# psteinb/libmultiviewnative

Hardware: AMD Instinct MI355X
Metric: RL iterations/sec on 512^3 f32, 6 views (higher is better)
Workload: dtype f32

## Files before the change

### libmultiviewnative_amd/csrc/mvn_backend_emu.cpp

```cpp
#ifndef MVN_HOST_EMU
#error "mvn_backend_emu.cpp is only for the MVN_HOST_EMU test build"
#endif

#include <atomic>
#include <chrono>
#include <cstdlib>
#include <cstring>
#include <map>
#include <memory>
#include <mutex>
#include <stdexcept>
#include <string>
#include <vector>

#include "mvn_backend.hpp"
#include "mvn_fixed_geom.hpp"
#include "mvn_wave_rows.hpp"

namespace mvn {
namespace be {

#define MVN_DISPATCH_T(T_, CALL)                                   \
  switch (T_) {                                                    \
    case 16: { constexpr int TT = 16; CALL; } break;               \
// ... 181 lines not shown
          case MVN_EPI_DIVIDE: fx_rows_run<H, 1, MVN_EPI_DIVIDE, Ctx, true>(p, t, ntiles, l, *ctx); break;
          case MVN_EPI_UPDATE: fx_rows_run<H, 1, MVN_EPI_UPDATE, Ctx, true>(p, t, ntiles, l, *ctx); break;
          case MVN_EPI_UPDATE_STATS: fx_rows_run_stats<H, 1, SCtx, true>(p, t, ntiles, l, *sctx); break;
          case MVN_EPI_DELTA: fx_rows_run<H, 1, MVN_EPI_DELTA, Ctx, true>(p, t, ntiles, l, *ctx); break;
          default: fx_rows_run<H, 1, MVN_EPI_STORE, Ctx, true>(p, t, ntiles, l, *ctx); break;
        }
      } else {
        switch (p.epi.mode) {
          case MVN_EPI_DIVIDE: fx_rows_run<H, 2, MVN_EPI_DIVIDE, Ctx, true>(p, t, ntiles, l, *ctx); break;
          case MVN_EPI_UPDATE: fx_rows_run<H, 2, MVN_EPI_UPDATE, Ctx, true>(p, t, ntiles, l, *ctx); break;
          case MVN_EPI_UPDATE_STATS: fx_rows_run_stats<H, 2, SCtx, true>(p, t, ntiles, l, *sctx); break;
          default: fx_rows_run<H, 2, MVN_EPI_STORE, Ctx, true>(p, t, ntiles, l, *ctx); break;
        }
      }
    }
  }
}

static std::atomic<long> g_mid_fused_launches{0};
long mid_fused_launch_count() { return g_mid_fused_launches.load(); }

template <int K>
static void emu_mid_fused(const MidFusedParams& p) {
  typedef FxCtx<MfRegs<K>, MF_NT> Ctx;
  const long blocks = mf_blocks(p);
#pragma omp parallel
  {
    std::vector<cfloat> lds(MF_LDS_CFLOATS + 8);
    std::unique_ptr<Ctx> ctx(new Ctx());
#pragma omp for schedule(static)
    for (long b = 0; b < blocks; ++b) mf_body<K>(p, b, lds.data(), *ctx);
  }
}
#define MVN_MF_TAP_COUNTS(X) X(1) X(3) X(5) X(7) X(9) X(11) X(13) X(15) X(17) X(19) X(21) X(23) X(25) X(27) X(29) X(31)
void launch_mid_fused(const MidFusedParams& p, stream_t) {
  mf_check(p);
  if (p.mode == MF_TAPS) {
    typedef FxCtx<MfRegs<1>, MF_NT> Ctx;
    const long blocks = mf_blocks(p);
#pragma omp parallel
    {
      std::vector<cfloat> lds(MF_LDS_CFLOATS + 8);
      std::unique_ptr<Ctx> ctx(new Ctx());
#pragma omp for schedule(static)
      for (long b = 0; b < blocks; ++b) mf_taps_body(p, b, lds.data(), *ctx);
    }
    return;
// ... 362 lines not shown
```

### libmultiviewnative_amd/csrc/mvn_kernels.hip

```cpp
#include <hip/hip_runtime.h>

#include <atomic>
#include <cstdio>
#include <cstdlib>
#include <cstring>
#include <map>
#include <mutex>
#include <tuple>
#include <stdexcept>
#include <string>

#include "mvn_backend.hpp"
#include "mvn_fixed_geom.hpp"
#include "mvn_wave_rows.hpp"

#define HIP_CHECK(expr)                                                                      \
  do {                                                                                       \
    hipError_t _e = (expr);                                                                  \
    if (_e != hipSuccess)                                                                    \
      throw std::runtime_error(std::string("HIP error '") + hipGetErrorString(_e) + "' at " + \
                               __FILE__ + ":" + std::to_string(__LINE__) + " (" #expr ")");  \
  } while (0)

template <bool EVEN, int T>
// ... 63 lines not shown
  Ctx ctx;
  ctx.tid = (int)threadIdx.x;
  if constexpr (EPI == MVN_EPI_UPDATE_STATS)
    fx_rows_run_stats<H, 1, Ctx, LINES>(p, (long)blockIdx.x, (long)gridDim.x, (cfloat*)mvn_smem, ctx);
  else
    fx_rows_run<H, 1, EPI, Ctx, LINES>(p, (long)blockIdx.x, (long)gridDim.x, (cfloat*)mvn_smem, ctx);
}

template <int H, int EPI, bool LINES = false>
__global__ void __launch_bounds__(FxRowsCfg<H>::NT) kx_rows_c2r_r2c(const RowsParams p0) {
  extern __shared__ __attribute__((aligned(16))) char mvn_smem[];
  RowsParams p = p0;
  mvn_arm_poison(p.epi);
  typedef FxCtx<FxRowsRegsFor<H, EPI>, FxRowsCfg<H>::NT> Ctx;
  Ctx ctx;
  ctx.tid = (int)threadIdx.x;
  if constexpr (EPI == MVN_EPI_UPDATE_STATS)
    fx_rows_run_stats<H, 2, Ctx, LINES>(p, (long)blockIdx.x, (long)gridDim.x, (cfloat*)mvn_smem, ctx);
  else
    fx_rows_run<H, 2, EPI, Ctx, LINES>(p, (long)blockIdx.x, (long)gridDim.x, (cfloat*)mvn_smem, ctx);
}

template <int K>
__global__ void __launch_bounds__(MF_NT) kf_mid(const MidFusedParams p) {
  extern __shared__ __attribute__((aligned(16))) char mvn_smem[];
  FxCtx<MfRegs<K>, MF_NT> ctx;
  ctx.tid = (int)threadIdx.x;
  mf_body<K>(p, (long)blockIdx.x, (cfloat*)mvn_smem, ctx);
}
__global__ void __launch_bounds__(MF_NT) kf_mid_taps(const MidFusedParams p) {
  extern __shared__ __attribute__((aligned(16))) char mvn_smem[];
  FxCtx<MfRegs<1>, MF_NT> ctx;
  ctx.tid = (int)threadIdx.x;
  mf_taps_body(p, (long)blockIdx.x, (cfloat*)mvn_smem, ctx);
}

template <int MODE, int EPI>
__global__ void __launch_bounds__(WrCfg::NT, 4) kw_rows(const RowsParams p0) {
  extern __shared__ __attribute__((aligned(16))) char mvn_smem[];
  RowsParams p = p0;
  if (MODE != MVN_WR_R2C) mvn_arm_poison(p.epi);
  FxCtx<WrRegs, WrCfg::NT> ctx;
  ctx.tid = (int)threadIdx.x;
  wr_rows_body<MODE, EPI>(p, (long)blockIdx.x, (long)gridDim.x, (cfloat*)mvn_smem, ctx);
}

template <int N, int MODE>
__global__ void __launch_bounds__((FxStridedSel<N, MODE>::NT), (FxStridedSel<N, MODE>::WAVES))
    kx_strided(const StridedParams p, const StridedParams rider, unsigned main_grid) {
// ... 653 lines not shown
  }
  if (nblocks > 0x7fffffffL) throw std::invalid_argument("mvn: grid size out of range");
  switch (mvn_dim0_taps_template(p.k)) {
#define X(K) case K: hipLaunchKernelGGL(kd_dim0<K>, dim3((unsigned)nblocks), dim3(MVN_D0_WG), lds, hs(s), p, (unsigned)main_blocks); break;
    MVN_D0_TAP_COUNTS(X)
#undef X
    default: throw std::invalid_argument("mvn: no direct dim0 kernel for this tap count");
  }
  HIP_CHECK(hipGetLastError());
}

#define MVN_MF_TAP_COUNTS(X) X(1) X(3) X(5) X(7) X(9) X(11) X(13) X(15) X(17) X(19) X(21) X(23) X(25) X(27) X(29) X(31)
void launch_mid_fused(const MidFusedParams& p, stream_t s) {
  mf_check(p);
  const long nblocks = mf_blocks(p);
  if (nblocks < 1 || nblocks > 0x7fffffffL) throw std::invalid_argument("mvn: grid size out of range");
  const size_t lds = sizeof(cfloat) * (size_t)MF_LDS_CFLOATS;
  if (p.mode == MF_TAPS) {
    launch_pass(kf_mid_taps, p, nblocks, MF_NT, lds, s);
    return;
  }
  ++g_mid_fused_launches;
  switch (mvn_dim0_taps_template(p.k)) {
#define X(K) case K: launch_pass(kf_mid<K>, p, nblocks, MF_NT, lds, s); break;
    MVN_MF_TAP_COUNTS(X)
#undef X
    default: throw std::invalid_argument("mvn: no fused middle pass for this tap count");
  }
}

static unsigned flat_grid(size_t n, int block) {
  size_t g = (n + (size_t)block - 1) / (size_t)block;
  const size_t cap = (size_t)device_cu_count() * 8;
  if (g > cap) g = cap;
  if (g < 1) g = 1;
  return (unsigned)g;
}

void launch_scatter_psf(const float* kernel, int k0, int k1, int k2, float* target, int D0,
                        int D1, int D2, long pitch, float scale, stream_t s) {
  const size_t total = (size_t)k0 * k1 * k2;
  hipLaunchKernelGGL(k_scatter_psf, dim3(flat_grid(total, 256)), dim3(256), 0, hs(s), kernel, k0,
                     k1, k2, target, D0, D1, D2, pitch, scale);
  HIP_CHECK(hipGetLastError());
}

void launch_copy3d(float* dst, long drow, long dplane, const float* src, long srow, long splane,
// ... 55 lines not shown
```

### libmultiviewnative_amd/csrc/mvn_mid_fused.hpp

```cpp
#pragma once

#include <stdexcept>

#include "mvn_dim0_direct.hpp"
#include "mvn_wave_rows.hpp"

#if defined(__HIPCC__) && !defined(MVN_HOST_EMU)
#define MF_WPHASE(ctx, ...)                                         \
  {                                                                 \
    const int tid = (ctx).tid;                                      \
    auto& r = (ctx).regs;                                           \
    (void)r;                                                        \
    __VA_ARGS__;                                                    \
  }                                                                 \
  __builtin_amdgcn_fence(__ATOMIC_SEQ_CST, "wavefront", "local");   \
  __builtin_amdgcn_wave_barrier();
#else
#define MF_WPHASE(ctx, ...) MVN_PHASE(ctx, __VA_ARGS__)
#endif

#define MF_N1 512
#define MF_NT 512
#define MF_LINES 8
#define MF_PITCH 576
#define MF_BUF (MF_LINES * MF_PITCH)
#define MF_TWL 512
#define MF_LDS_CFLOATS (4 * MF_BUF + MF_TWL)

struct MidFusedParams {
  const cfloat* in;
  cfloat* out;
  const cfloat* taps;
  int kd;
  const cfloat* tw;
  int d0, H;
  int k, h;
  int seg;
  int mode;
  int packed;
  int zbeg, zcount;
  unsigned* poison;
  unsigned poison_epoch;
  int n_peers;
  unsigned* const* poison_peers;
};
enum { MF_CONV = 0, MF_TAPS = 1 };
enum { MF_DC_NONE = 0, MF_DC_LOW = 1, MF_DC_HIGH = 2, MF_DC_SELF = 3 };

constexpr int mf_slots(int K) { return (K + 7) / 8 * 8; }

template <int K>
struct MfRegs {
  cfloat tap[K];
  cfloat w[mf_slots(K)];
  cfloat xr[8];
  cfloat t[8];
  cfloat bad;
  cfloat t2[8];
  cfloat xn[2], xp[2];
  int dcmode, qm, cpar;
};

inline long mf_pieces(const MidFusedParams& P) { return (P.seg > 0 && P.zcount <= 0) ? (P.d0 + P.seg - 1) / P.seg : 1; }
inline long mf_blocks(const MidFusedParams& P) { return P.mode == MF_TAPS ? (long)P.H * ((P.d0 + MF_LINES - 1) / MF_LINES) : (long)P.H * mf_pieces(P); }

MVN_HD void mf_job(const MidFusedParams& P, long block, int& c, int& z0, int& nout) {
  const long piece = block / P.H;
  c = (int)(block - piece * P.H);
  if (P.zcount > 0) {
    z0 = P.zbeg;
    nout = P.zcount;
  } else if (P.seg > 0) {
    z0 = (int)(piece * P.seg);
    nout = P.d0 - z0 < P.seg ? P.d0 - z0 : P.seg;
  } else {
    z0 = 0;
    nout = P.d0;
  }
}

MVN_HD int mf_tap_plane(const MidFusedParams& P, int j) {
  const int p = j - P.h;
  return p < 0 ? p + P.kd : p;
}

inline void mf_check(const MidFusedParams& P) {
  const bool taps_mode = P.mode == MF_TAPS;
  if (!P.in || !P.out || !P.tw || P.d0 < 1 || P.H < 1 || (long)P.d0 * P.H * MF_N1 >= (1L << 31) * 4 || P.seg < 0)
    throw std::invalid_argument("mvn: fused middle pass: bad arguments");
  if (P.zcount < 0 || P.zbeg < 0 || P.zbeg + P.zcount > P.d0 || P.n_peers < 0 || P.n_peers > MVN_D0_MAX_PEERS ||
      (P.n_peers > 0 && !P.poison_peers))
    throw std::invalid_argument("mvn: fused middle pass: bad plane range or peers");
  if (!taps_mode && (!P.taps || P.in == P.out || P.k < 1 || mvn_dim0_taps_template(P.k) > 31 || P.h != P.k / 2 || P.kd < P.k))
    throw std::invalid_argument("mvn: fused middle pass called outside its range");
}

MVN_HD int mf_in_plane(const MidFusedParams& P, int z0, int n) {
  int z = (z0 - P.h + n) % P.d0;
  return z < 0 ? z + P.d0 : z;
}

template <int K>
MVN_HD void mf_fetch(const MidFusedParams& P, MfRegs<K>& r, int c, int z0, int batch, int nsteps, int tid) {
  const int wv = tid >> 6, l = tid & 63;
  const int n = batch * MF_LINES + wv;
  if (n >= nsteps) return;
  const cfloat* src = P.in + ((long)mf_in_plane(P, z0, n) * P.H + c) * MF_N1 + l;
#pragma unroll
  for (int m = 0; m < 8; ++m) r.xr[m] = src[64 * m];
}

template <int K>
MVN_HD void mf_setup(const MidFusedParams& P, MfRegs<K>& r, int c, int z0, int nsteps, int tid) {
  r.bad = cmake(0.f, 0.f);
  r.dcmode = MF_DC_NONE;
  r.qm = r.cpar = 0;
#pragma unroll
  for (int j = 0; j < K; ++j) r.tap[j] = j < P.k ? P.taps[((long)mf_tap_plane(P, j) * P.H + c) * MF_N1 + tid] : cmake(0.f, 0.f);
#pragma unroll
  for (int s = 0; s < mf_slots(K); ++s) r.w[s] = cmake(0.f, 0.f);
  mf_fetch<K>(P, r, c, z0, 0, nsteps, tid);
}

MVN_HD cfloat mf_cmul(cfloat a, cfloat w) {
#if defined(MVN_PACKED)
  cfloat t, r;
  MVN_PK2(t, "v_pk_mul_f32", a, w, "op_sel_hi:[0,1]");
  MVN_PK3(r, "v_pk_fma_f32", a, w, t, "op_sel:[1,1,0] op_sel_hi:[1,0,1] neg_lo:[0,1,0]");
  return r;
#else
  return cmul(a, w);
#endif
}
MVN_HD cfloat mf_cmulc(cfloat a, cfloat w) {
#if defined(MVN_PACKED)
  cfloat t, r;
  MVN_PK2(t, "v_pk_mul_f32", a, w, "op_sel_hi:[0,1] neg_hi:[0,1]");
  MVN_PK3(r, "v_pk_fma_f32", a, w, t, "op_sel:[1,1,0] op_sel_hi:[1,0,1]");
  return r;
#else
  return cmulc(a, w);
#endif
}

MVN_HD void mf_build_twiddles(const MidFusedParams& P, cfloat* twl, int tid) {
  if (tid < 448) {
    const int m = tid / 64 + 1, l = tid & 63;
    twl[tid] = P.tw[l * m];
  } else if (tid < 448 + 56) {
    const int e = tid - 448, m = e / 8 + 1, j = e & 7;
    twl[tid] = P.tw[8 * j * m];
  }
}
MVN_HD cfloat mf_tw0(const cfloat* twl, int l, int m) { return twl[(m - 1) * 64 + l]; }
MVN_HD cfloat mf_tw1(const cfloat* twl, int l, int m) { return twl[448 + (m - 1) * 8 + (l & 7)]; }

template <int K>
MVN_HD void mf_fwd0(MfRegs<K>& r, cfloat* buf, int tid) {
  const int wv = tid >> 6, l = tid & 63;
  cfloat* line = buf + wv * MF_PITCH;
  cfloat a[8];
#pragma unroll
  for (int m = 0; m < 8; ++m) a[m] = r.xr[m];
  dftR<8, -1>(a);
#pragma unroll
  for (int m = 1; m < 8; ++m) a[m] = mf_cmul(a[m], r.t2[m]);
#pragma unroll
  for (int m = 0; m < 8; ++m) line[72 * m + l] = a[m];
}
template <int K>
MVN_HD void mf_tw0_ahead(MfRegs<K>& r, const cfloat* twl, int tid) {
  const int l = tid & 63;
#pragma unroll
  for (int m = 1; m < 8; ++m) r.t2[m] = mf_tw0(twl, l, m);
}
template <int K>
MVN_HD void mf_fwd1_r(MfRegs<K>& r, const cfloat* buf, int tid) {
  const int wv = tid >> 6, l = tid & 63;
  const cfloat* p = buf + wv * MF_PITCH + 72 * (l >> 3) + (l & 7);
#pragma unroll
  for (int m = 0; m < 8; ++m) r.t[m] = p[8 * m];
}
template <int K>
MVN_HD void mf_fwd1_c(MfRegs<K>& r, const cfloat* twl, int tid) {
  const int l = tid & 63;
  (void)l;
  dftR<8, -1>(r.t);
#pragma unroll
  for (int m = 1; m < 8; ++m) r.t[m] = mf_cmul(r.t[m], mf_tw1(twl, l, m));
}
template <int K>
MVN_HD void mf_fwd1_r2(MfRegs<K>& r, const cfloat* buf, int tid) {
  const int wv = tid >> 6, l = tid & 63;
  const cfloat* p = buf + wv * MF_PITCH + 72 * (l >> 3) + (l & 7);
#pragma unroll
  for (int m = 0; m < 8; ++m) r.t2[m] = p[8 * m];
}
template <int K>
MVN_HD void mf_fwd1_c2(MfRegs<K>& r, const cfloat* twl, int tid) {
  const int l = tid & 63;
  (void)l;
  dftR<8, -1>(r.t2);
#pragma unroll
  for (int m = 1; m < 8; ++m) r.t2[m] = mf_cmul(r.t2[m], mf_tw1(twl, l, m));
}
template <int K>
MVN_HD void mf_fwd1_b2(const MfRegs<K>& r, cfloat* buf, int tid) {
  const int wv = tid >> 6, l = tid & 63;
  cfloat* p = buf + wv * MF_PITCH + 72 * (l >> 3) + (l & 7);
#pragma unroll
  for (int m = 0; m < 8; ++m) p[9 * m] = r.t2[m];
}
template <int K>
MVN_HD void mf_fwd2_r2(MfRegs<K>& r, const cfloat* buf, int tid) {
  const int wv = tid >> 6, l = tid & 63;
  const cfloat* p = buf + wv * MF_PITCH + 72 * (l >> 3) + 9 * (l & 7);
#pragma unroll
  for (int m = 0; m < 8; ++m) r.t2[m] = p[m];
}
template <int K>
MVN_HD void mf_fwd2_b2(const MfRegs<K>& r, cfloat* buf, int tid) {
  const int wv = tid >> 6, l = tid & 63;
  cfloat* line = buf + wv * MF_PITCH;
#pragma unroll
  for (int m = 0; m < 8; ++m) line[64 * m + l] = r.t2[m];
}
template <int K>
MVN_HD void mf_fwd1_a(MfRegs<K>& r, const cfloat* buf, const cfloat* twl, int tid) {
  mf_fwd1_r<K>(r, buf, tid);
  mf_fwd1_c<K>(r, twl, tid);
}
template <int K>
MVN_HD void mf_fwd1_b(const MfRegs<K>& r, cfloat* buf, int tid) {
  const int wv = tid >> 6, l = tid & 63;
  cfloat* p = buf + wv * MF_PITCH + 72 * (l >> 3) + (l & 7);
#pragma unroll
  for (int m = 0; m < 8; ++m) p[9 * m] = r.t[m];
}
template <int K>
MVN_HD void mf_fwd2_r(MfRegs<K>& r, const cfloat* buf, int tid) {
  const int wv = tid >> 6, l = tid & 63;
  const cfloat* p = buf + wv * MF_PITCH + 72 * (l >> 3) + 9 * (l & 7);
#pragma unroll
  for (int m = 0; m < 8; ++m) r.t[m] = p[m];
}
template <int K>
MVN_HD void mf_fwd2_a(MfRegs<K>& r, const cfloat* buf, int tid) {
  mf_fwd2_r<K>(r, buf, tid);
  dftR<8, -1>(r.t);
}
// ... 46 lines not shown
}
template <int K>
MVN_HD void mf_inv1_b(const MfRegs<K>& r, cfloat* buf, int tid) {
  const int wv = tid >> 6, l = tid & 63;
  cfloat* p = buf + wv * MF_PITCH + 72 * (l >> 3) + (l & 7);
#pragma unroll
  for (int m = 0; m < 8; ++m) p[8 * m] = r.t[m];
}
template <int K>
MVN_HD void mf_inv0_r(MfRegs<K>& r, const cfloat* buf, int tid) {
  const int wv = tid >> 6, l = tid & 63;
  const cfloat* line = buf + wv * MF_PITCH;
#pragma unroll
  for (int m = 0; m < 8; ++m) r.t[m] = line[72 * m + l];
}
template <int K>
MVN_HD void mf_inv0_c_store(MfRegs<K>& r, const cfloat* twl, cfloat* dst, int tid) {
  const int l = tid & 63;
#pragma unroll
  for (int m = 1; m < 8; ++m) r.t[m] = mf_cmulc(r.t[m], mf_tw0(twl, l, m));
  dftR<8, +1>(r.t);
#pragma unroll
  for (int m = 0; m < 8; ++m) dst[l + 64 * m] = r.t[m];
}
template <int K>
MVN_HD void mf_inv0_store(MfRegs<K>& r, const cfloat* buf, const cfloat* twl, cfloat* dst, int tid) {
  mf_inv0_r<K>(r, buf, tid);
  mf_inv0_c_store<K>(r, twl, dst, tid);
}

template <int K>
MVN_HD void mf_store_line(const MidFusedParams& P, MfRegs<K>& r, const cfloat* buf, const cfloat* twl, int c, int z0,
                          int nout, int batch, int tid) {
  const int m = batch * MF_LINES + (tid >> 6) - (K - 1);
  if (m < 0 || m >= nout) return;
  int z = z0 + m;
  z = z >= P.d0 ? z - P.d0 : z;
  mf_inv0_store<K>(r, buf, twl, P.out + ((long)z * P.H + c) * MF_N1, tid);
}
template <int K>
MVN_HD void mf_store_line_c(const MidFusedParams& P, MfRegs<K>& r, const cfloat* twl, int c, int z0, int nout, int batch,
                            int tid) {
  const int m = batch * MF_LINES + (tid >> 6) - (K - 1);
  if (m < 0 || m >= nout) return;
  int z = z0 + m;
  z = z >= P.d0 ? z - P.d0 : z;
  mf_inv0_c_store<K>(r, twl, P.out + ((long)z * P.H + c) * MF_N1, tid);
}

MVN_HD int mf_bin_of(int f) { return 64 * (f >> 6) + 8 * (f & 7) + ((f >> 3) & 7); }
MVN_HD int mf_freq_of(int q) { return ((q >> 3) & 7) + 8 * (q & 7) + 64 * (q >> 6); }
MVN_HD cfloat mf_herm0(cfloat a, cfloat b) { return cmake(0.5f * (a.x + b.x), 0.5f * (a.y - b.y)); }
MVN_HD cfloat mf_hermh(cfloat a, cfloat b) { return cmake(0.5f * (a.y + b.y), 0.5f * (b.x - a.x)); }


template <int K>
MVN_HD void mf_setup_dc(const MidFusedParams& P, MfRegs<K>& r, int tid) {
  const int f = mf_freq_of(tid), fm = (MF_N1 - f) & (MF_N1 - 1);
  r.qm = mf_bin_of(fm);
  r.dcmode = f == fm ? MF_DC_SELF : (f < MF_N1 / 2 ? MF_DC_LOW : MF_DC_HIGH);
  {
    const int l = tid & 63, g = (l >> 3) + 8 * (l & 7);
    r.cpar = g == 0 ? 64 : 8 * ((64 - g) & 7) + ((64 - g) >> 3);
  }
  const cfloat* tp = P.taps + r.qm;
#pragma unroll
  for (int j = 0; j < K; ++j) {
    const cfloat a = r.tap[j], b = j < P.k ? tp[(long)mf_tap_plane(P, j) * P.H * MF_N1] : cmake(0.f, 0.f);
    r.tap[j] = f == fm ? a : (f < MF_N1 / 2 ? mf_herm0(a, b) : mf_hermh(b, a));
  }
}

template <int K>
MVN_HD void mf_fread(MfRegs<K>& r, const cfloat* in, int c, bool dc, int tid) {
  r.xn[c & 1] = in[c * MF_PITCH + tid];
  if (dc) r.xp[c & 1] = in[c * MF_PITCH + r.qm];
}
template <int K>
MVN_HD cfloat mf_filter_input(MfRegs<K>& r, int c, bool dc) {
  cfloat x = r.xn[c & 1];
  if (dc) {
    const cfloat xp = r.xp[c & 1];
    const cfloat lo = mf_herm0(x, xp), hi = mf_hermh(xp, x);
    x = r.dcmode == MF_DC_LOW ? lo : (r.dcmode == MF_DC_HIGH ? hi : x);
  }
  return x;
}
template <int K, int U, int C, bool FILL>
MVN_HD void mf_filter_line(MfRegs<K>& r, const cfloat* in, cfloat* out, bool dc, int tid) {
  constexpr int KW = mf_slots(K), S = 8 * U + C;
  if (FILL) {
    r.w[S] = mf_filter_input<K>(r, C, dc);
    return;
  }
  constexpr int NC = K < 4 ? K : 4;
  cfloat a1[NC], a2[NC];
#pragma unroll
  for (int j = K - 1; j >= 1; --j) {
    const int ch = j % NC;
    const bool first = j + NC > K - 1;
    if (first)
      mvn_cmul2(a1[ch], a2[ch], r.w[(S - j + 2 * KW) % KW], r.tap[j]);
    else
      mvn_cmac2(a1[ch], a2[ch], r.w[(S - j + 2 * KW) % KW], r.tap[j]);
  }
  const cfloat x = mf_filter_input<K>(r, C, dc);
  if (K <= NC)
    mvn_cmul2(a1[0], a2[0], x, r.tap[0]);
  else
    mvn_cmac2(a1[0], a2[0], x, r.tap[0]);
  cfloat s1 = a1[0], s2 = a2[0];
#pragma unroll
  for (int ch = 1; ch < NC; ++ch) {
    s1 = cadd(s1, a1[ch]);
    s2 = cadd(s2, a2[ch]);
  }
  r.w[S] = x;
  r.bad = mvn_dim0_track(r.bad, x);
  cfloat o = cadd_i<+1>(s1, s2);
  if (dc) o = r.dcmode == MF_DC_SELF ? cmake(s1.x, s2.y) : o;
  out[C * MF_PITCH + tid] = o;
}
template <int K, int C>
MVN_HD void mf_fread_ahead(MfRegs<K>& r, const cfloat* in, bool dc, int tid) {
  if (C + 1 < MF_LINES) mf_fread<K>(r, in, C + 1, dc, tid);
}
template <int K, int C, int U>
MVN_HD void mf_fline_dispatch(MfRegs<K>& r, const cfloat* in, cfloat* out, int u, bool fill, bool dc, int tid) {
  if (u == U) {
    if (fill)
      mf_filter_line<K, U, C, true>(r, in, out, dc, tid);
    else
      mf_filter_line<K, U, C, false>(r, in, out, dc, tid);
    return;
  }
  if constexpr (U + 1 < mf_slots(K) / 8) mf_fline_dispatch<K, C, U + 1>(r, in, out, u, fill, dc, tid);
}

template <int K>
MVN_HD void mf_inv2_fix_dc(MfRegs<K>& r, const cfloat* buf, int tid) {
  const int wv = tid >> 6, l = tid & 63;
  const cfloat* line = buf + wv * MF_PITCH;
#pragma unroll
  for (int m = 0; m < 8; ++m) {
    const cfloat o = r.t[m];
    const cfloat p = line[(64 * (7 - m) + r.cpar) & (MF_N1 - 1)];
    const cfloat low = cmake(o.x - p.y, o.y + p.x), high = cmake(p.x + o.y, o.x - p.y);
    cfloat v = m < 4 ? low : high;
    if (m == 0 || m == 4) v = l == 0 ? o : v;
    r.t[m] = v;
  }
}
template <int K>
MVN_HD void mf_inv2_r_dc(MfRegs<K>& r, const cfloat* buf, int tid) {
  mf_inv2_r<K>(r, buf, tid);
  mf_inv2_fix_dc<K>(r, buf, tid);
}

template <int K>
MVN_HD void mf_report(const MidFusedParams& P, const MfRegs<K>& r) {
  if (r.bad.x != 0.f || r.bad.y != 0.f) {
    if (P.poison) *P.poison = P.poison_epoch;
    for (int i = 0; i < P.n_peers; ++i) *P.poison_peers[i] = P.poison_epoch;
  }
}

template <int K, typename Ctx>
MVN_HD void mf_body(const MidFusedParams& P, long block, cfloat* lds, Ctx& ctx) {
  constexpr int NT_ = MF_NT;
  (void)NT_;
  int c, z0, nout;
  mf_job(P, block, c, z0, nout);
  const int nsteps = nout + K - 1;
  const int nb = (nsteps + MF_LINES - 1) / MF_LINES;
  const bool dc = P.packed && c == 0;
  cfloat* twl = lds + 4 * MF_BUF;
  MVN_PHASE_NOSYNC(ctx, (mf_setup<K>(P, r, c, z0, nsteps, tid), mf_build_twiddles(P, twl, tid)));
  if (dc) {
    MVN_PHASE_NOSYNC(ctx, (mf_setup_dc<K>(P, r, tid)));
  }
  MVN_PHASE(ctx, (void)0);
  MVN_PHASE_NOSYNC(ctx, (mf_tw0_ahead<K>(r, twl, tid)));
#if defined(__HIPCC__) && !defined(MVN_HOST_EMU)
  const int wave_young = mvn_uniform((ctx.tid >> 8) & 1);
#define MF_PRIO_RESET() __builtin_amdgcn_s_setprio(0);
#define MF_PRIO_RAISE_YOUNG() \
  if (wave_young != 0) __builtin_amdgcn_s_setprio(2);
#else
#define MF_PRIO_RESET()
#define MF_PRIO_RAISE_YOUNG()
#endif
  for (int i = -1; i <= nb; ++i) {
    const cfloat* fin = lds + (i & 1) * MF_BUF;
    cfloat* fout = lds + (2 + (i & 1)) * MF_BUF;
    cfloat* fwd = lds + ((i + 1) & 1) * MF_BUF;
    cfloat* inv = lds + (2 + ((i + 1) & 1)) * MF_BUF;
    const bool F = i >= 0 && i < nb;
    const bool fill = i * MF_LINES + MF_LINES - 1 < K - 1;
    const int u = F ? i % (mf_slots(K) / 8) : 0;
#define MF_FLINE(C)                                                                \
  if (F) {                                                                         \
    MF_WPHASE(ctx, (mf_fread_ahead<K, C>(r, fin, dc, tid), mf_fline_dispatch<K, C, 0>(r, fin, fout, u, fill, dc, tid)));  \
  }
    MF_PRIO_RESET()
    if (F) {
      MF_WPHASE(ctx, (mf_fread<K>(r, fin, 0, dc, tid)));
    }
    MF_WPHASE(ctx, (mf_inv2_r<K>(r, inv, tid)));
    if (dc) {
      MF_WPHASE(ctx, (mf_inv2_fix_dc<K>(r, inv, tid)));
    }
    MF_WPHASE(ctx, (mf_fwd0<K>(r, fwd, tid), mf_fetch<K>(P, r, c, z0, i + 2, nsteps, tid)));
    MF_FLINE(0)
    MF_WPHASE(ctx, (dftR<8, +1>(r.t), mf_inv2_b<K>(r, inv, tid)));
    MF_WPHASE(ctx, (mf_inv1_r<K>(r, inv, tid)));
    MF_WPHASE(ctx, (mf_fwd1_r2<K>(r, fwd, tid)));
    MF_FLINE(1)
    MF_FLINE(2)
    MF_PRIO_RAISE_YOUNG()
    MF_WPHASE(ctx, (mf_inv1_c<K>(r, twl, tid), mf_inv1_b<K>(r, inv, tid)));
    MF_WPHASE(ctx, (mf_fwd1_c2<K>(r, twl, tid), mf_fwd1_b2<K>(r, fwd, tid)));
    MF_WPHASE(ctx, (mf_inv0_r<K>(r, inv, tid)));
    MF_WPHASE(ctx, (mf_fwd2_r2<K>(r, fwd, tid)));
    MF_FLINE(3)
    MF_FLINE(4)
    MF_WPHASE(ctx, (mf_store_line_c<K>(P, r, twl, c, z0, nout, i - 1, tid)));
    MF_WPHASE(ctx, (dftR<8, -1>(r.t2), mf_fwd2_b2<K>(r, fwd, tid)));
    MF_FLINE(5)
    MF_FLINE(6)
    MF_FLINE(7)
#undef MF_FLINE
    MF_WPHASE(ctx, (mf_tw0_ahead<K>(r, twl, tid)));
    MVN_PHASE(ctx, (void)0);
  }
#undef MF_PRIO_RESET
#undef MF_PRIO_RAISE_YOUNG
  MVN_PHASE_NOSYNC(ctx, (mf_report<K>(P, r)));
}

MVN_HD void mf_taps_load(const MidFusedParams& P, MfRegs<1>& r, long batch, int c, int tid) {
  const int l = tid & 63, z = (int)batch * MF_LINES + (tid >> 6);
  if (z >= P.d0) return;
  const cfloat* src = P.in + ((long)z * P.H + c) * MF_N1 + l;
#pragma unroll
  for (int m = 0; m < 8; ++m) r.xr[m] = src[64 * m];
}
MVN_HD void mf_taps_store(const MidFusedParams& P, const cfloat* lds, long batch, int c, int tid) {
  const int l = tid & 63, wv = tid >> 6, z = (int)batch * MF_LINES + wv;
  if (z >= P.d0) return;
  cfloat* dst = P.out + ((long)z * P.H + c) * MF_N1 + l;
#pragma unroll
  for (int m = 0; m < 8; ++m) dst[64 * m] = lds[wv * MF_PITCH + 64 * m + l];
}
template <typename Ctx>
MVN_HD void mf_taps_body(const MidFusedParams& P, long block, cfloat* lds, Ctx& ctx) {
  constexpr int NT_ = MF_NT;
  (void)NT_;
  const long batch = block / P.H;
  const int c = (int)(block - batch * P.H);
  cfloat* twl = lds + 4 * MF_BUF;
  MVN_PHASE(ctx, (mf_taps_load(P, r, batch, c, tid), mf_build_twiddles(P, twl, tid)));
  MF_WPHASE(ctx, (mf_tw0_ahead<1>(r, twl, tid)));
  MF_WPHASE(ctx, (mf_fwd0<1>(r, lds, tid)));
  MF_WPHASE(ctx, (mf_fwd1_a<1>(r, lds, twl, tid)));
  MF_WPHASE(ctx, (mf_fwd1_b<1>(r, lds, tid)));
  MF_WPHASE(ctx, (mf_fwd2_a<1>(r, lds, tid)));
  MF_WPHASE(ctx, (mf_fwd2_b<1>(r, lds, tid)));
  MVN_PHASE_NOSYNC(ctx, (mf_taps_store(P, lds, batch, c, tid)));
}
```

Baseline: 103.3.

## Split fused middle pass into forward and inverse warp roles with 1024 threads

```diff
diff --git a/libmultiviewnative_amd/csrc/mvn_backend_emu.cpp b/libmultiviewnative_amd/csrc/mvn_backend_emu.cpp
--- a/libmultiviewnative_amd/csrc/mvn_backend_emu.cpp
+++ b/libmultiviewnative_amd/csrc/mvn_backend_emu.cpp
@@ -227,7 +227,7 @@
 
 template <int K>
 static void emu_mid_fused(const MidFusedParams& p) {
-  typedef FxCtx<MfRegs<K>, MF_NT> Ctx;
+  typedef FxCtx<MfRegs<K>, MF_NTC> Ctx;
   const long blocks = mf_blocks(p);
 #pragma omp parallel
   {
diff --git a/libmultiviewnative_amd/csrc/mvn_kernels.hip b/libmultiviewnative_amd/csrc/mvn_kernels.hip
--- a/libmultiviewnative_amd/csrc/mvn_kernels.hip
+++ b/libmultiviewnative_amd/csrc/mvn_kernels.hip
@@ -109,9 +109,9 @@
 }
 
 template <int K>
-__global__ void __launch_bounds__(MF_NT) kf_mid(const MidFusedParams p) {
-  extern __shared__ __attribute__((aligned(16))) char mvn_smem[];
-  FxCtx<MfRegs<K>, MF_NT> ctx;
+__global__ void __launch_bounds__(MF_NTC) kf_mid(const MidFusedParams p) {
+  extern __shared__ __attribute__((aligned(16))) char mvn_smem[];
+  FxCtx<MfRegs<K>, MF_NTC> ctx;
   ctx.tid = (int)threadIdx.x;
   mf_body<K>(p, (long)blockIdx.x, (cfloat*)mvn_smem, ctx);
 }
@@ -811,7 +811,7 @@
   }
   ++g_mid_fused_launches;
   switch (mvn_dim0_taps_template(p.k)) {
-#define X(K) case K: launch_pass(kf_mid<K>, p, nblocks, MF_NT, lds, s); break;
+#define X(K) case K: launch_pass(kf_mid<K>, p, nblocks, MF_NTC, lds, s); break;
     MVN_MF_TAP_COUNTS(X)
 #undef X
     default: throw std::invalid_argument("mvn: no fused middle pass for this tap count");
diff --git a/libmultiviewnative_amd/csrc/mvn_mid_fused.hpp b/libmultiviewnative_amd/csrc/mvn_mid_fused.hpp
--- a/libmultiviewnative_amd/csrc/mvn_mid_fused.hpp
+++ b/libmultiviewnative_amd/csrc/mvn_mid_fused.hpp
@@ -21,6 +21,7 @@
 
 #define MF_N1 512
 #define MF_NT 512
+#define MF_NTC 1024
 #define MF_LINES 8
 #define MF_PITCH 576
 #define MF_BUF (MF_LINES * MF_PITCH)
@@ -47,18 +48,23 @@
 enum { MF_CONV = 0, MF_TAPS = 1 };
 enum { MF_DC_NONE = 0, MF_DC_LOW = 1, MF_DC_HIGH = 2, MF_DC_SELF = 3 };
 
-constexpr int mf_slots(int K) { return (K + 7) / 8 * 8; }
+constexpr int mf_ring(int K) {
+  const int kh = (K + 1) / 2;
+  return kh <= 2 ? kh : (kh <= 4 ? 4 : (kh <= 6 ? 6 : (kh <= 8 ? 8 : (kh <= 12 ? 12 : 16))));
+}
+constexpr int mf_gcd8(int R) { return R % 8 == 0 ? 8 : (R % 4 == 0 ? 4 : (R % 2 == 0 ? 2 : 1)); }
+constexpr int mf_variants(int K) { return mf_ring(K) / mf_gcd8(mf_ring(K)); }
 
 template <int K>
 struct MfRegs {
-  cfloat tap[K];
-  cfloat w[mf_slots(K)];
+  cfloat tap[mf_ring(K)];
+  cfloat acc[mf_ring(K)];
   cfloat xr[8];
   cfloat t[8];
   cfloat bad;
-  cfloat t2[8];
   cfloat xn[2], xp[2];
-  int dcmode, qm, cpar;
+  cfloat hand;
+  int qm;
 };
 
 inline long mf_pieces(const MidFusedParams& P) { return (P.seg > 0 && P.zcount <= 0) ? (P.d0 + P.seg - 1) / P.seg : 1; }
@@ -103,8 +109,8 @@
 template <int K>
 MVN_HD void mf_fetch(const MidFusedParams& P, MfRegs<K>& r, int c, int z0, int batch, int nsteps, int tid) {
   const int wv = tid >> 6, l = tid & 63;
-  const int n = batch * MF_LINES + wv;
-  if (n >= nsteps) return;
+  int n = batch * MF_LINES + wv;
+  n = n < nsteps ? n : nsteps - 1;
   const cfloat* src = P.in + ((long)mf_in_plane(P, z0, n) * P.H + c) * MF_N1 + l;
 #pragma unroll
   for (int m = 0; m < 8; ++m) r.xr[m] = src[64 * m];
@@ -112,14 +118,16 @@
 
 template <int K>
 MVN_HD void mf_setup(const MidFusedParams& P, MfRegs<K>& r, int c, int z0, int nsteps, int tid) {
+  constexpr int R = mf_ring(K);
+  const int q = tid >> 1, j0 = (tid & 1) * R;
   r.bad = cmake(0.f, 0.f);
-  r.dcmode = MF_DC_NONE;
-  r.qm = r.cpar = 0;
-#pragma unroll
-  for (int j = 0; j < K; ++j) r.tap[j] = j < P.k ? P.taps[((long)mf_tap_plane(P, j) * P.H + c) * MF_N1 + tid] : cmake(0.f, 0.f);
-#pragma unroll
-  for (int s = 0; s < mf_slots(K); ++s) r.w[s] = cmake(0.f, 0.f);
-  mf_fetch<K>(P, r, c, z0, 0, nsteps, tid);
+  r.hand = cmake(0.f, 0.f);
+  r.qm = 0;
+#pragma unroll
+  for (int i = 0; i < R; ++i)
+    r.tap[i] = j0 + i < P.k ? P.taps[((long)mf_tap_plane(P, j0 + i) * P.H + c) * MF_N1 + q] : cmake(0.f, 0.f);
+#pragma unroll
+  for (int s = 0; s < R; ++s) r.acc[s] = cmake(0.f, 0.f);
 }
 
 MVN_HD cfloat mf_cmul(cfloat a, cfloat w) {
@@ -156,23 +164,16 @@
 MVN_HD cfloat mf_tw1(const cfloat* twl, int l, int m) { return twl[448 + (m - 1) * 8 + (l & 7)]; }
 
 template <int K>
-MVN_HD void mf_fwd0(MfRegs<K>& r, cfloat* buf, int tid) {
+MVN_HD void mf_fwd0(MfRegs<K>& r, cfloat* buf, const cfloat* twl, int tid) {
   const int wv = tid >> 6, l = tid & 63;
   cfloat* line = buf + wv * MF_PITCH;
-  cfloat a[8];
-#pragma unroll
-  for (int m = 0; m < 8; ++m) a[m] = r.xr[m];
-  dftR<8, -1>(a);
-#pragma unroll
-  for (int m = 1; m < 8; ++m) a[m] = mf_cmul(a[m], r.t2[m]);
-#pragma unroll
-  for (int m = 0; m < 8; ++m) line[72 * m + l] = a[m];
-}
-template <int K>
-MVN_HD void mf_tw0_ahead(MfRegs<K>& r, const cfloat* twl, int tid) {
-  const int l = tid & 63;
-#pragma unroll
-  for (int m = 1; m < 8; ++m) r.t2[m] = mf_tw0(twl, l, m);
+#pragma unroll
+  for (int m = 0; m < 8; ++m) r.t[m] = r.xr[m];
+  dftR<8, -1>(r.t);
+#pragma unroll
+  for (int m = 1; m < 8; ++m) r.t[m] = mf_cmul(r.t[m], mf_tw0(twl, l, m));
+#pragma unroll
+  for (int m = 0; m < 8; ++m) line[72 * m + l] = r.t[m];
 }
 template <int K>
 MVN_HD void mf_fwd1_r(MfRegs<K>& r, const cfloat* buf, int tid) {
@@ -190,42 +191,6 @@
   for (int m = 1; m < 8; ++m) r.t[m] = mf_cmul(r.t[m], mf_tw1(twl, l, m));
 }
 template <int K>
-MVN_HD void mf_fwd1_r2(MfRegs<K>& r, const cfloat* buf, int tid) {
-  const int wv = tid >> 6, l = tid & 63;
-  const cfloat* p = buf + wv * MF_PITCH + 72 * (l >> 3) + (l & 7);
-#pragma unroll
-  for (int m = 0; m < 8; ++m) r.t2[m] = p[8 * m];
-}
-template <int K>
-MVN_HD void mf_fwd1_c2(MfRegs<K>& r, const cfloat* twl, int tid) {
-  const int l = tid & 63;
-  (void)l;
-  dftR<8, -1>(r.t2);
-#pragma unroll
-  for (int m = 1; m < 8; ++m) r.t2[m] = mf_cmul(r.t2[m], mf_tw1(twl, l, m));
-}
-template <int K>
-MVN_HD void mf_fwd1_b2(const MfRegs<K>& r, cfloat* buf, int tid) {
-  const int wv = tid >> 6, l = tid & 63;
-  cfloat* p = buf + wv * MF_PITCH + 72 * (l >> 3) + (l & 7);
-#pragma unroll
-  for (int m = 0; m < 8; ++m) p[9 * m] = r.t2[m];
-}
-template <int K>
-MVN_HD void mf_fwd2_r2(MfRegs<K>& r, const cfloat* buf, int tid) {
-  const int wv = tid >> 6, l = tid & 63;
-  const cfloat* p = buf + wv * MF_PITCH + 72 * (l >> 3) + 9 * (l & 7);
-#pragma unroll
-  for (int m = 0; m < 8; ++m) r.t2[m] = p[m];
-}
-template <int K>
-MVN_HD void mf_fwd2_b2(const MfRegs<K>& r, cfloat* buf, int tid) {
-  const int wv = tid >> 6, l = tid & 63;
-  cfloat* line = buf + wv * MF_PITCH;
-#pragma unroll
-  for (int m = 0; m < 8; ++m) line[64 * m + l] = r.t2[m];
-}
-template <int K>
 MVN_HD void mf_fwd1_a(MfRegs<K>& r, const cfloat* buf, const cfloat* twl, int tid) {
   mf_fwd1_r<K>(r, buf, tid);
   mf_fwd1_c<K>(r, twl, tid);
@@ -318,21 +283,6 @@
   dftR<8, +1>(r.t);
 #pragma unroll
   for (int m = 0; m < 8; ++m) dst[l + 64 * m] = r.t[m];
-}
-template <int K>
-MVN_HD void mf_inv0_store(MfRegs<K>& r, const cfloat* buf, const cfloat* twl, cfloat* dst, int tid) {
-  mf_inv0_r<K>(r, buf, tid);
-  mf_inv0_c_store<K>(r, twl, dst, tid);
-}
-
-template <int K>
-MVN_HD void mf_store_line(const MidFusedParams& P, MfRegs<K>& r, const cfloat* buf, const cfloat* twl, int c, int z0,
-                          int nout, int batch, int tid) {
-  const int m = batch * MF_LINES + (tid >> 6) - (K - 1);
-  if (m < 0 || m >= nout) return;
-  int z = z0 + m;
-  z = z >= P.d0 ? z - P.d0 : z;
-  mf_inv0_store<K>(r, buf, twl, P.out + ((long)z * P.H + c) * MF_N1, tid);
 }
 template <int K>
 MVN_HD void mf_store_line_c(const MidFusedParams& P, MfRegs<K>& r, const cfloat* twl, int c, int z0, int nout, int batch,
@@ -346,112 +296,128 @@
 
 MVN_HD int mf_bin_of(int f) { return 64 * (f >> 6) + 8 * (f & 7) + ((f >> 3) & 7); }
 MVN_HD int mf_freq_of(int q) { return ((q >> 3) & 7) + 8 * (q & 7) + 64 * (q >> 6); }
+MVN_HD int mf_dcmode(int q) { return (q & (MF_N1 / 2 - 1)) == 0 ? MF_DC_SELF : (q < MF_N1 / 2 ? MF_DC_LOW : MF_DC_HIGH); }
 MVN_HD cfloat mf_herm0(cfloat a, cfloat b) { return cmake(0.5f * (a.x + b.x), 0.5f * (a.y - b.y)); }
 MVN_HD cfloat mf_hermh(cfloat a, cfloat b) { return cmake(0.5f * (a.y + b.y), 0.5f * (b.x - a.x)); }
 
 
 template <int K>
 MVN_HD void mf_setup_dc(const MidFusedParams& P, MfRegs<K>& r, int tid) {
-  const int f = mf_freq_of(tid), fm = (MF_N1 - f) & (MF_N1 - 1);
+  constexpr int R = mf_ring(K);
+  const int q = tid >> 1, j0 = (tid & 1) * R;
+  const int f = mf_freq_of(q), fm = (MF_N1 - f) & (MF_N1 - 1);
   r.qm = mf_bin_of(fm);
-  r.dcmode = f == fm ? MF_DC_SELF : (f < MF_N1 / 2 ? MF_DC_LOW : MF_DC_HIGH);
-  {
-    const int l = tid & 63, g = (l >> 3) + 8 * (l & 7);
-    r.cpar = g == 0 ? 64 : 8 * ((64 - g) & 7) + ((64 - g) >> 3);
-  }
   const cfloat* tp = P.taps + r.qm;
 #pragma unroll
-  for (int j = 0; j < K; ++j) {
-    const cfloat a = r.tap[j], b = j < P.k ? tp[(long)mf_tap_plane(P, j) * P.H * MF_N1] : cmake(0.f, 0.f);
-    r.tap[j] = f == fm ? a : (f < MF_N1 / 2 ? mf_herm0(a, b) : mf_hermh(b, a));
+  for (int i = 0; i < R; ++i) {
+    const int j = j0 + i;
+    const cfloat a = r.tap[i], b = j < P.k ? tp[(long)mf_tap_plane(P, j) * P.H * MF_N1] : cmake(0.f, 0.f);
+    r.tap[i] = f == fm ? a : (f < MF_N1 / 2 ? mf_herm0(a, b) : mf_hermh(b, a));
   }
 }
 
 template <int K>
 MVN_HD void mf_fread(MfRegs<K>& r, const cfloat* in, int c, bool dc, int tid) {
-  r.xn[c & 1] = in[c * MF_PITCH + tid];
+  r.xn[c & 1] = in[c * MF_PITCH + (tid >> 1)];
   if (dc) r.xp[c & 1] = in[c * MF_PITCH + r.qm];
 }
 template <int K>
-MVN_HD cfloat mf_filter_input(MfRegs<K>& r, int c, bool dc) {
+MVN_HD cfloat mf_filter_input(MfRegs<K>& r, int c, bool dc, int tid) {
   cfloat x = r.xn[c & 1];
   if (dc) {
+    const int dcmode = mf_dcmode(tid >> 1);
     const cfloat xp = r.xp[c & 1];
     const cfloat lo = mf_herm0(x, xp), hi = mf_hermh(xp, x);
-    x = r.dcmode == MF_DC_LOW ? lo : (r.dcmode == MF_DC_HIGH ? hi : x);
+    x = dcmode == MF_DC_LOW ? lo : (dcmode == MF_DC_HIGH ? hi : x);
   }
   return x;
 }
-template <int K, int U, int C, bool FILL>
-MVN_HD void mf_filter_line(MfRegs<K>& r, const cfloat* in, cfloat* out, bool dc, int tid) {
-  constexpr int KW = mf_slots(K), S = 8 * U + C;
-  if (FILL) {
-    r.w[S] = mf_filter_input<K>(r, C, dc);
-    return;
-  }
-  constexpr int NC = K < 4 ? K : 4;
-  cfloat a1[NC], a2[NC];
-#pragma unroll
-  for (int j = K - 1; j >= 1; --j) {
-    const int ch = j % NC;
-    const bool first = j + NC > K - 1;
-    if (first)
-      mvn_cmul2(a1[ch], a2[ch], r.w[(S - j + 2 * KW) % KW], r.tap[j]);
-    else
-      mvn_cmac2(a1[ch], a2[ch], r.w[(S - j + 2 * KW) % KW], r.tap[j]);
-  }
-  const cfloat x = mf_filter_input<K>(r, C, dc);
-  if (K <= NC)
-    mvn_cmul2(a1[0], a2[0], x, r.tap[0]);
-  else
-    mvn_cmac2(a1[0], a2[0], x, r.tap[0]);
-  cfloat s1 = a1[0], s2 = a2[0];
-#pragma unroll
-  for (int ch = 1; ch < NC; ++ch) {
-    s1 = cadd(s1, a1[ch]);
-    s2 = cadd(s2, a2[ch]);
-  }
-  r.w[S] = x;
-  r.bad = mvn_dim0_track(r.bad, x);
-  cfloat o = cadd_i<+1>(s1, s2);
-  if (dc) o = r.dcmode == MF_DC_SELF ? cmake(s1.x, s2.y) : o;
-  out[C * MF_PITCH + tid] = o;
+MVN_HD void mf_mac_re(cfloat& acc, cfloat x, cfloat w) {
+#if defined(MVN_PACKED)
+  asm("v_pk_fma_f32 %0, %1, %2, %0 op_sel_hi:[0,1,1]" : "+v"(acc) : "v"(x), "v"(w));
+#else
+  acc = cmake(acc.x + x.x * w.x, acc.y + x.x * w.y);
+#endif
+}
+MVN_HD void mf_mac_im(cfloat& acc, cfloat x, cfloat w) {
+#if defined(MVN_PACKED)
+  asm("v_pk_fma_f32 %0, %1, %2, %0 op_sel:[1,1,0] op_sel_hi:[1,0,1] neg_lo:[0,1,0]" : "+v"(acc) : "v"(x), "v"(w));
+#else
+  acc = cmake(acc.x - x.y * w.y, acc.y + x.y * w.x);
+#endif
+}
+MVN_HD void mf_mac_p1(cfloat& acc, cfloat p1, cfloat w) {
+#if defined(MVN_PACKED)
+  asm("v_pk_fma_f32 %0, %1, %2, %0" : "+v"(acc) : "v"(p1), "v"(w));
+#else
+  acc = cmake(acc.x + p1.x * w.x, acc.y + p1.y * w.y);
+#endif
+}
+MVN_HD void mf_mac_p2(cfloat& acc, cfloat p2, cfloat w) {
+#if defined(MVN_PACKED)
+  asm("v_pk_fma_f32 %0, %1, %2, %0 op_sel:[0,1,0] op_sel_hi:[1,0,1] neg_lo:[0,1,0]" : "+v"(acc) : "v"(p2), "v"(w));
+#else
+  acc = cmake(acc.x - p2.x * w.y, acc.y + p2.y * w.x);
+#endif
+}
+template <int K, int S>
+MVN_HD void mf_handoff(MfRegs<K>& r, int tid) {
+#if defined(MVN_PACKED)
+  const cfloat a = r.acc[S];
+  const float mx = __int_as_float(__builtin_amdgcn_update_dpp(0, __float_as_int(a.x), 0xF5, 0xF, 0xF, false));
+  const float my = __int_as_float(__builtin_amdgcn_update_dpp(0, __float_as_int(a.y), 0xF5, 0xF, 0xF, false));
+  r.acc[S] = (tid & 1) ? cmake(0.f, 0.f) : cmake(mx, my);
+#else
+  r.acc[S] = (tid & 1) ? cmake(0.f, 0.f) : (&r)[1].hand;
+#endif
+}
+template <int K, int S, int C, bool DC, int PART>
+MVN_HD void mf_filter_line(MfRegs<K>& r, cfloat* out, bool track, int tid) {
+  constexpr int R = mf_ring(K);
+  if (PART != 1) {
+    const cfloat x = mf_filter_input<K>(r, C, DC, tid);
+    if (DC) {
+      const bool self = mf_dcmode(tid >> 1) == MF_DC_SELF;
+      const cfloat p1 = self ? x : cmake(x.x, x.x), p2 = self ? cmake(0.f, 0.f) : cmake(x.y, x.y);
+#pragma unroll
+      for (int i = 0; i < R; ++i) mf_mac_p1(r.acc[(S + i) % R], p1, r.tap[i]);
+#pragma unroll
+      for (int i = 0; i < R; ++i) mf_mac_p2(r.acc[(S + i) % R], p2, r.tap[i]);
+    } else {
+#pragma unroll
+      for (int i = 0; i < R; ++i) mf_mac_re(r.acc[(S + i) % R], x, r.tap[i]);
+#pragma unroll
+      for (int i = 0; i < R; ++i) mf_mac_im(r.acc[(S + i) % R], x, r.tap[i]);
+    }
+    if (track) r.bad = mvn_dim0_track(r.bad, x);
+    if ((tid & 1) == 0) out[C * MF_PITCH + (tid >> 1)] = r.acc[S];
+#if !defined(MVN_PACKED)
+    r.hand = r.acc[S];
+#endif
+  }
+  if (PART != 0) mf_handoff<K, S>(r, tid);
 }
 template <int K, int C>
 MVN_HD void mf_fread_ahead(MfRegs<K>& r, const cfloat* in, bool dc, int tid) {
   if (C + 1 < MF_LINES) mf_fread<K>(r, in, C + 1, dc, tid);
 }
-template <int K, int C, int U>
-MVN_HD void mf_fline_dispatch(MfRegs<K>& r, const cfloat* in, cfloat* out, int u, bool fill, bool dc, int tid) {
-  if (u == U) {
-    if (fill)
-      mf_filter_line<K, U, C, true>(r, in, out, dc, tid);
-    else
-      mf_filter_line<K, U, C, false>(r, in, out, dc, tid);
-    return;
-  }
-  if constexpr (U + 1 < mf_slots(K) / 8) mf_fline_dispatch<K, C, U + 1>(r, in, out, u, fill, dc, tid);
-}
 
 template <int K>
 MVN_HD void mf_inv2_fix_dc(MfRegs<K>& r, const cfloat* buf, int tid) {
   const int wv = tid >> 6, l = tid & 63;
   const cfloat* line = buf + wv * MF_PITCH;
+  const int g = (l >> 3) + 8 * (l & 7);
+  const int cpar = g == 0 ? 64 : 8 * ((64 - g) & 7) + ((64 - g) >> 3);
 #pragma unroll
   for (int m = 0; m < 8; ++m) {
     const cfloat o = r.t[m];
-    const cfloat p = line[(64 * (7 - m) + r.cpar) & (MF_N1 - 1)];
+    const cfloat p = line[(64 * (7 - m) + cpar) & (MF_N1 - 1)];
     const cfloat low = cmake(o.x - p.y, o.y + p.x), high = cmake(p.x + o.y, o.x - p.y);
     cfloat v = m < 4 ? low : high;
     if (m == 0 || m == 4) v = l == 0 ? o : v;
     r.t[m] = v;
   }
 }
-template <int K>
-MVN_HD void mf_inv2_r_dc(MfRegs<K>& r, const cfloat* buf, int tid) {
-  mf_inv2_r<K>(r, buf, tid);
-  mf_inv2_fix_dc<K>(r, buf, tid);
-}
 
 template <int K>
 MVN_HD void mf_report(const MidFusedParams& P, const MfRegs<K>& r) {
@@ -461,9 +427,123 @@
   }
 }
 
+#if defined(__HIPCC__) && !defined(MVN_HOST_EMU)
+#define MF_RPHASE(ctx, LO, ...) MF_WPHASE(ctx, __VA_ARGS__)
+#else
+#define MF_RPHASE(ctx, LO, ...)                         \
+  for (int tid = (LO); tid < (LO) + MF_NT; ++tid) {     \
+    auto& r = (ctx).regs[tid];                          \
+    (void)r;                                            \
+    __VA_ARGS__;                                        \
+  }
+#endif
+
+template <int K, int ROLE, bool DC, int U, typename Ctx>
+MVN_HD void mf_iter(const MidFusedParams& P, cfloat* lds, Ctx& ctx, int i, int nb, int c, int z0, int nout, int nsteps) {
+  constexpr bool dc = DC;
+  constexpr int LO = ROLE * MF_NT;
+  cfloat* twl = lds + 4 * MF_BUF;
+  const cfloat* fin = lds + (i & 1) * MF_BUF;
+  cfloat* fout = lds + (2 + (i & 1)) * MF_BUF;
+  cfloat* fwd = lds + ((i + 1) & 1) * MF_BUF;
+  cfloat* inv = lds + (2 + ((i + 1) & 1)) * MF_BUF;
+  (void)fwd, (void)inv, (void)nsteps, (void)nout;
+  const bool F = i >= 0 && i < nb;
+  const bool track = !(i * MF_LINES + MF_LINES - 1 < K - 1);
+#if defined(__HIPCC__) && !defined(MVN_HOST_EMU)
+#define MF_FLINE(C)                                                                                                     \
+  if (F) {                                                                                                              \
+    MF_RPHASE(ctx, LO, (mf_fread_ahead<K, C>(r, fin, dc, tid), mf_filter_line<K, (8 * U + C) % mf_ring(K), C, DC, 2>(r, fout, track, tid))); \
+  }
+#else
+#define MF_FLINE(C)                                                                                                     \
+  if (F) {                                                                                                              \
+    MF_RPHASE(ctx, LO, (mf_fread_ahead<K, C>(r, fin, dc, tid), mf_filter_line<K, (8 * U + C) % mf_ring(K), C, DC, 0>(r, fout, track, tid))); \
+    MF_RPHASE(ctx, LO, (mf_filter_line<K, (8 * U + C) % mf_ring(K), C, DC, 1>(r, fout, track, tid)));                                    \
+  }
+#endif
+#define MF_FREAD0()                                          \
+  if (F) {                                                   \
+    MF_RPHASE(ctx, LO, (mf_fread<K>(r, fin, 0, dc, tid)));   \
+  }
+  if (ROLE == 0) {
+    MF_RPHASE(ctx, LO, (mf_fwd0<K>(r, fwd, twl, tid - LO), mf_fetch<K>(P, r, c, z0, i + 2, nsteps, tid - LO)));
+    MF_FREAD0()
+    MF_FLINE(0)
+    MF_FLINE(1)
+    MF_RPHASE(ctx, LO, (mf_fwd1_r<K>(r, fwd, tid - LO)));
+    MF_FLINE(2)
+    MF_FLINE(3)
+    MF_RPHASE(ctx, LO, (mf_fwd1_c<K>(r, twl, tid - LO), mf_fwd1_b<K>(r, fwd, tid - LO)));
+    MF_RPHASE(ctx, LO, (mf_fwd2_r<K>(r, fwd, tid - LO)));
+    MF_FLINE(4)
+    MF_FLINE(5)
+    MF_RPHASE(ctx, LO, (dftR<8, -1>(r.t), mf_fwd2_b<K>(r, fwd, tid - LO)));
+    MF_FLINE(6)
+    MF_FLINE(7)
+  } else {
+    MF_RPHASE(ctx, LO, (mf_inv2_r<K>(r, inv, tid - LO)));
+    if (dc) {
+      MF_RPHASE(ctx, LO, (mf_inv2_fix_dc<K>(r, inv, tid - LO)));
+    }
+    MF_FREAD0()
+    MF_FLINE(0)
+    MF_FLINE(1)
+    MF_RPHASE(ctx, LO, (dftR<8, +1>(r.t), mf_inv2_b<K>(r, inv, tid - LO)));
+    MF_RPHASE(ctx, LO, (mf_inv1_r<K>(r, inv, tid - LO)));
+    MF_FLINE(2)
+    MF_FLINE(3)
+    MF_RPHASE(ctx, LO, (mf_inv1_c<K>(r, twl, tid - LO), mf_inv1_b<K>(r, inv, tid - LO)));
+    MF_RPHASE(ctx, LO, (mf_inv0_r<K>(r, inv, tid - LO)));
+    MF_FLINE(4)
+    MF_FLINE(5)
+    MF_RPHASE(ctx, LO, (mf_store_line_c<K>(P, r, twl, c, z0, nout, i - 1, tid - LO)));
+    MF_FLINE(6)
+    MF_FLINE(7)
+  }
+#undef MF_FLINE
+#undef MF_FREAD0
+}
+
+template <int K, int ROLE, bool DC, int U, typename Ctx>
+MVN_HD void mf_group(const MidFusedParams& P, cfloat* lds, Ctx& ctx, int i0, int nb, int c, int z0, int nout, int nsteps) {
+  const int i = i0 + U;
+  if (i >= -1 && i <= nb) {
+#if defined(__HIPCC__) && !defined(MVN_HOST_EMU)
+    mf_iter<K, ROLE, DC, U>(P, lds, ctx, i, nb, c, z0, nout, nsteps);
+    MVN_PHASE(ctx, (void)0);
+#else
+    mf_iter<K, 0, DC, U>(P, lds, ctx, i, nb, c, z0, nout, nsteps);
+    mf_iter<K, 1, DC, U>(P, lds, ctx, i, nb, c, z0, nout, nsteps);
+#endif
+  }
+  if constexpr (U + 1 < mf_variants(K)) mf_group<K, ROLE, DC, U + 1>(P, lds, ctx, i0, nb, c, z0, nout, nsteps);
+}
+template <int K, bool DC, typename Ctx>
+MVN_HD void mf_walk(const MidFusedParams& P, cfloat* lds, Ctx& ctx, int nb, int c, int z0, int nout, int nsteps) {
+  constexpr int V = mf_variants(K);
+#if defined(__HIPCC__) && !defined(MVN_HOST_EMU)
+  if (mvn_uniform(ctx.tid >> 9) == 0) {
+    MVN_PHASE_NOSYNC(ctx, (mf_fetch<K>(P, r, c, z0, 0, nsteps, tid)));
+    for (int i0 = -V; i0 <= nb; i0 += V) {
+      MVN_TILE_LOOP_TOP(ctx);
+      mf_group<K, 0, DC, 0>(P, lds, ctx, i0, nb, c, z0, nout, nsteps);
+    }
+  } else {
+    for (int i0 = -V; i0 <= nb; i0 += V) {
+      MVN_TILE_LOOP_TOP(ctx);
+      mf_group<K, 1, DC, 0>(P, lds, ctx, i0, nb, c, z0, nout, nsteps);
+    }
+  }
+#else
+  MF_RPHASE(ctx, 0, (mf_fetch<K>(P, r, c, z0, 0, nsteps, tid)));
+  for (int i0 = -V; i0 <= nb; i0 += V) mf_group<K, 0, DC, 0>(P, lds, ctx, i0, nb, c, z0, nout, nsteps);
+#endif
+}
+
 template <int K, typename Ctx>
 MVN_HD void mf_body(const MidFusedParams& P, long block, cfloat* lds, Ctx& ctx) {
-  constexpr int NT_ = MF_NT;
+  constexpr int NT_ = MF_NTC;
   (void)NT_;
   int c, z0, nout;
   mf_job(P, block, c, z0, nout);
@@ -476,61 +556,10 @@
     MVN_PHASE_NOSYNC(ctx, (mf_setup_dc<K>(P, r, tid)));
   }
   MVN_PHASE(ctx, (void)0);
-  MVN_PHASE_NOSYNC(ctx, (mf_tw0_ahead<K>(r, twl, tid)));
-#if defined(__HIPCC__) && !defined(MVN_HOST_EMU)
-  const int wave_young = mvn_uniform((ctx.tid >> 8) & 1);
-#define MF_PRIO_RESET() __builtin_amdgcn_s_setprio(0);
-#define MF_PRIO_RAISE_YOUNG() \
-  if (wave_young != 0) __builtin_amdgcn_s_setprio(2);
-#else
-#define MF_PRIO_RESET()
-#define MF_PRIO_RAISE_YOUNG()
-#endif
-  for (int i = -1; i <= nb; ++i) {
-    const cfloat* fin = lds + (i & 1) * MF_BUF;
-    cfloat* fout = lds + (2 + (i & 1)) * MF_BUF;
-    cfloat* fwd = lds + ((i + 1) & 1) * MF_BUF;
-    cfloat* inv = lds + (2 + ((i + 1) & 1)) * MF_BUF;
-    const bool F = i >= 0 && i < nb;
-    const bool fill = i * MF_LINES + MF_LINES - 1 < K - 1;
-    const int u = F ? i % (mf_slots(K) / 8) : 0;
-#define MF_FLINE(C)                                                                \
-  if (F) {                                                                         \
-    MF_WPHASE(ctx, (mf_fread_ahead<K, C>(r, fin, dc, tid), mf_fline_dispatch<K, C, 0>(r, fin, fout, u, fill, dc, tid)));  \
-  }
-    MF_PRIO_RESET()
-    if (F) {
-      MF_WPHASE(ctx, (mf_fread<K>(r, fin, 0, dc, tid)));
-    }
-    MF_WPHASE(ctx, (mf_inv2_r<K>(r, inv, tid)));
-    if (dc) {
-      MF_WPHASE(ctx, (mf_inv2_fix_dc<K>(r, inv, tid)));
-    }
-    MF_WPHASE(ctx, (mf_fwd0<K>(r, fwd, tid), mf_fetch<K>(P, r, c, z0, i + 2, nsteps, tid)));
-    MF_FLINE(0)
-    MF_WPHASE(ctx, (dftR<8, +1>(r.t), mf_inv2_b<K>(r, inv, tid)));
-    MF_WPHASE(ctx, (mf_inv1_r<K>(r, inv, tid)));
-    MF_WPHASE(ctx, (mf_fwd1_r2<K>(r, fwd, tid)));
-    MF_FLINE(1)
-    MF_FLINE(2)
-    MF_PRIO_RAISE_YOUNG()
-    MF_WPHASE(ctx, (mf_inv1_c<K>(r, twl, tid), mf_inv1_b<K>(r, inv, tid)));
-    MF_WPHASE(ctx, (mf_fwd1_c2<K>(r, twl, tid), mf_fwd1_b2<K>(r, fwd, tid)));
-    MF_WPHASE(ctx, (mf_inv0_r<K>(r, inv, tid)));
-    MF_WPHASE(ctx, (mf_fwd2_r2<K>(r, fwd, tid)));
-    MF_FLINE(3)
-    MF_FLINE(4)
-    MF_WPHASE(ctx, (mf_store_line_c<K>(P, r, twl, c, z0, nout, i - 1, tid)));
-    MF_WPHASE(ctx, (dftR<8, -1>(r.t2), mf_fwd2_b2<K>(r, fwd, tid)));
-    MF_FLINE(5)
-    MF_FLINE(6)
-    MF_FLINE(7)
-#undef MF_FLINE
-    MF_WPHASE(ctx, (mf_tw0_ahead<K>(r, twl, tid)));
-    MVN_PHASE(ctx, (void)0);
-  }
-#undef MF_PRIO_RESET
-#undef MF_PRIO_RAISE_YOUNG
+  if (dc)
+    mf_walk<K, true>(P, lds, ctx, nb, c, z0, nout, nsteps);
+  else
+    mf_walk<K, false>(P, lds, ctx, nb, c, z0, nout, nsteps);
   MVN_PHASE_NOSYNC(ctx, (mf_report<K>(P, r)));
 }
 
@@ -556,8 +585,7 @@
   const int c = (int)(block - batch * P.H);
   cfloat* twl = lds + 4 * MF_BUF;
   MVN_PHASE(ctx, (mf_taps_load(P, r, batch, c, tid), mf_build_twiddles(P, twl, tid)));
-  MF_WPHASE(ctx, (mf_tw0_ahead<1>(r, twl, tid)));
-  MF_WPHASE(ctx, (mf_fwd0<1>(r, lds, tid)));
+  MF_WPHASE(ctx, (mf_fwd0<1>(r, lds, twl, tid)));
   MF_WPHASE(ctx, (mf_fwd1_a<1>(r, lds, twl, tid)));
   MF_WPHASE(ctx, (mf_fwd1_b<1>(r, lds, tid)));
   MF_WPHASE(ctx, (mf_fwd2_a<1>(r, lds, tid)));
```

Measured after the change: 100.6. 0.974x the previous value.
